# 6Lackiu/EMplanner_Carla

Measured on AMD Instinct MI355X. Metric: planning cycles/sec (DP+QP, 40x9 S-L lattice, 8 obs), higher is better.
Workload: dtype f64

## Files before the change

### emplanner_carla_amd/csrc/emp_dp_kernels.h

```cpp
#pragma once

#include <hip/hip_runtime.h>

#include "emp_core.h"
#include "emp_dp_launch.h"

namespace emp {

__device__ __forceinline__ double jerk_unit_sum(const double* tail, double s0) {
    Quintic u;
    u.a0 = u.a1 = u.a2 = 0.0;
    u.a3 = tail[kSamples + kSampleMoments + 0];
    u.a4 = tail[kSamples + kSampleMoments + 1];
    u.a5 = tail[kSamples + kSampleMoments + 2];
    return jerk_quirk_sum(u, s0, tail[kSamples], tail[kSamples + 1]);
}

__global__ __launch_bounds__(256) void dp_pair_table_kernel(DpDev P, double* __restrict__ tab) {
    const int row = P.row, rr = P.row * P.row;
    for (int p = threadIdx.x; p < rr; p += blockDim.x) {
        const int k = p / row, i = p - k * row;
        const double l_pre = lattice_l(row, k, P.sample_l);
        const double l_cur = lattice_l(row, i, P.sample_l);
        const Quintic q = quintic_shifted(l_pre, 0.0, 0.0, l_cur, P.sample_s);
        double S_l = 0.0, S_dl = 0.0, S_ddl = 0.0;
        for (int n = 0; n < kSamples; ++n) {
            const double t = sample_t(n, P.sample_s);
            const double l = quintic_l(q, t);
            const double dl = quintic_dl(q, t);
            const double ddl = quintic_ddl(q, t);
            tab[n * rr + p] = l;
            S_l = S_l + l * l;
            S_dl = S_dl + dl * dl;
            S_ddl = S_ddl + ddl * ddl;
        }
        const double h = l_cur - l_pre;
        tab[kF_JERK * rr + p] = P.w2 * (h * h);
        tab[kF_BASE * rr + p] = P.w0 * S_dl + P.w1 * S_ddl;
        tab[kF_REF * rr + p] = P.w_ref * S_l;
        tab[kF_LLO * rr + p] = fmin(l_pre, l_cur);
        tab[kF_LHI * rr + p] = fmax(l_pre, l_cur);
    }
    if (threadIdx.x < kSamples) tab[kTableFields * rr + threadIdx.x] = sample_t(threadIdx.x, P.sample_s);
    if (threadIdx.x == 0) {
        sample_moments(P.sample_s, &tab[kTableFields * rr + kSamples], &tab[kTableFields * rr + kSamples + 1]);
        const Quintic u = quintic_shifted(0.0, 0.0, 0.0, 1.0, P.sample_s);
        tab[kTableFields * rr + kSamples + kSampleMoments + 0] = u.a3;
        tab[kTableFields * rr + kSamples + kSampleMoments + 1] = u.a4;
        tab[kTableFields * rr + kSamples + kSampleMoments + 2] = u.a5;
    }
}

#ifndef EMP_SOFT_NEWTON_STEPS
#define EMP_SOFT_NEWTON_STEPS 1
#endif
__device__ __forceinline__ double soft_cost_quotient(double d2) {
    double r = __builtin_amdgcn_rcp(d2);
    r = __builtin_fma(r, __builtin_fma(-d2, r, 1.0), r);
    if (EMP_SOFT_NEWTON_STEPS > 1) r = __builtin_fma(r, __builtin_fma(-d2, r, 1.0), r);
    const double q = kSoftGain * r;
    return __builtin_fma(__builtin_fma(-d2, q, kSoftGain), r, q);
}

#ifndef EMP_SCAN_GROUP
#define EMP_SCAN_GROUP 10
#endif
__device__ __forceinline__ double obstacle_scan_dense(double s0, const double* t_smp, const double* l_n, int stride,
                                                      double os, double ol, double w_coll) {
    double c = 0.0;
    bool alive = true;
#pragma unroll
    for (int g = 0; g < kSamples; g += EMP_SCAN_GROUP) {
        double d2[EMP_SCAN_GROUP];
#pragma unroll
        for (int n = 0; n < EMP_SCAN_GROUP; ++n) {
            const double d_lon = os - (s0 + t_smp[g + n]);
            const double d_lat = ol - l_n[(g + n) * stride];
            d2[n] = d_lon * d_lon + d_lat * d_lat;
        }
#pragma unroll
        for (int n = 0; n < EMP_SCAN_GROUP; ++n) {
            const bool near = alive & (d2[n] < kSafe2);
            const bool hard = near & (d2[n] <= kDanger2);
            if (near & !hard) {
#if EMP_SOFT_NEWTON_STEPS == 1
                asm volatile("");
#endif
                c = c + soft_cost_quotient(d2[n]);
            }
            alive = alive & !hard;
        }
    }
    if (!alive) c = c + w_coll;
    return c;
}

__device__ __forceinline__ bool obstacle_box_in_reach(double os, double ol, double s0, double s9, double l_lo, double l_hi) {
    const double dx = fmax(fmax(s0 - os, os - s9), 0.0);
    const double dy = fmax(fmax(l_lo - ol, ol - l_hi), 0.0);
    return dx * dx + dy * dy < 36.5;
}

template <int ROW = 0, typename MASK = unsigned long long, typename Store>
__device__ __forceinline__ void dp_edge_column(const DpDev& P, int j, int i, double ps, int nob, const double* tab,
                                               const double* t_smp, const double* my_obs_s, const double* my_obs_l,
                                               Store&& store, double* box_dx2 = nullptr) {
    constexpr int kMaskBits = (int)sizeof(MASK) * 8;
    const int row = ROW > 0 ? ROW : P.row, rr = row * row;
    const int nmask = min(nob, kMaskBits);
    const double s0 = ps + (double)j * P.sample_s;
    const double s9 = s0 + t_smp[kSamples - 1];
    const double F = jerk_unit_sum(t_smp, s0);
    MASK near_s = 0;
    for (int m = 0; m < nmask; ++m) {
        const double os = my_obs_s[m];
        if (os > s0 - 6.5 && os < s9 + 6.5) near_s |= (MASK)1 << m;
    }
    if (box_dx2) {
        for (int m = i; m < nmask; m += row) {
            const double os = my_obs_s[m];
            const double dx = fmax(fmax(s0 - os, os - s9), 0.0);
            box_dx2[m] = dx * dx;
        }
        __builtin_amdgcn_wave_barrier();
    }
    for (int k = 0; k < row; ++k) {
        const int p = k * row + i;
        const double smooth = tab[kF_BASE * rr + p] + tab[kF_JERK * rr + p] * F;
        const double l_lo = tab[kF_LLO * rr + p], l_hi = tab[kF_LHI * rr + p];
        double coll = 0.0;
        for (MASK rest = near_s; rest; rest &= rest - 1) {
            const int m = (kMaskBits == 32 ? __ffs((int)rest) : __ffsll((long long)rest)) - 1;
            const double ol = my_obs_l[m];
            if (box_dx2) {
                const double dy = fmax(fmax(l_lo - ol, ol - l_hi), 0.0);
                if (!(box_dx2[m] + dy * dy < 36.5)) continue;
                coll = coll + obstacle_scan_dense(s0, t_smp, &tab[p], rr, my_obs_s[m], ol, P.w_coll);
                continue;
            }
            const double os = my_obs_s[m];
            if (!obstacle_box_in_reach(os, ol, s0, s9, l_lo, l_hi)) continue;
            coll = coll + obstacle_scan_dense(s0, t_smp, &tab[p], rr, os, ol, P.w_coll);
        }
        for (int m = kMaskBits; m < nob; ++m) {
            const double os = my_obs_s[m], ol = my_obs_l[m];
            if (!obstacle_in_reach(os, ol, s0, s9, l_lo, l_hi)) continue;
            coll = coll + obstacle_scan_dense(s0, t_smp, &tab[p], rr, os, ol, P.w_coll);
        }
        store(k, (smooth + coll) + tab[kF_REF * rr + p]);
    }
    if (box_dx2) __builtin_amdgcn_wave_barrier();
}

#ifndef EMP_EDGE_WAVES
#define EMP_EDGE_WAVES 5
#endif
template <bool TILED, int ROW = 0, typename MASK = unsigned long long>
__global__ __launch_bounds__(1024, EMP_EDGE_WAVES) void dp_edge_kernel(DpDev P, const double* __restrict__ pair_tab,
                                                      const double* __restrict__ obs_s,
                                                      const double* __restrict__ obs_l,
                                                      const int* __restrict__ n_obs,
                                                      const double* __restrict__ start,
                                                      double* __restrict__ start_cost,
                                                      double* __restrict__ edge, int cols_per_chunk) {
    extern __shared__ __attribute__((aligned(16))) double lds[];
    __builtin_amdgcn_s_setprio(EMP_PRIO_FRONT);
    const int row = ROW > 0 ? ROW : P.row, rr = row * row;
    double* tab = lds;
    double* t_obs_s = lds + kTableFields * rr;
    double* t_obs_l = t_obs_s + P.S * P.max_obs;
    double* t_smp = t_obs_l + P.S * P.max_obs;
    const int box_w = min(P.max_obs, (int)sizeof(MASK) * 8);
    double* box_all = t_smp + kTableTail;
    const int tile = blockIdx.x;
    const int tid = threadIdx.x;

    for (int x = tid; x < kTableFields * rr; x += blockDim.x) tab[x] = pair_tab[x];
    if (tid < kTableTail) t_smp[tid] = pair_tab[kTableFields * rr + tid];
    for (int x = tid; x < P.S * P.max_obs; x += blockDim.x) {
        const int s = x / P.max_obs, m = x - s * P.max_obs;
        const int b = tile * P.S + s;
        t_obs_s[x] = (b < P.B) ? obs_s[(size_t)b * P.max_obs + m] : 0.0;
        t_obs_l[x] = (b < P.B) ? obs_l[(size_t)b * P.max_obs + m] : 0.0;
    }
    __syncthreads();

    const int lanes_used = P.S * row;

    if (blockIdx.y == 0 && start_cost != nullptr && tid < lanes_used) {
        const int s = tid / row, i = tid - s * row;
        const int b = tile * P.S + s;
        if (b < P.B) {
            const double ps = start[b * 4 + 0], pl = start[b * 4 + 1], pdl = start[b * 4 + 2],
                         pddl = start[b * 4 + 3];
            const Quintic q = quintic_shifted(pl, pdl, pddl, lattice_l(row, i, P.sample_l), P.sample_s);
            start_cost[(size_t)b * row + i] =
                segment_cost(q, ps, P.sample_s, t_obs_s + s * P.max_obs, t_obs_l + s * P.max_obs, min(max(n_obs[b], 0), P.max_obs),
                             P.w_coll, P.w0, P.w1, P.w2, P.w_ref);
        }
    }

    const int j_begin = 1 + blockIdx.y * cols_per_chunk;
    const int j_end = min(P.col, j_begin + cols_per_chunk);
    const int lane = tid & 63;
    const int s = lane / row, i = lane - s * row;
    const int b = tile * P.S + s;
    if (lane >= lanes_used || b >= P.B) return;
    const double ps = start[b * 4 + 0];
    const int nob = min(max(n_obs[b], 0), P.max_obs);
    const double* my_obs_s = t_obs_s + s * P.max_obs;
    const double* my_obs_l = t_obs_l + s * P.max_obs;
    double* my_box = box_all + ((size_t)(tid >> 6) * P.S + s) * box_w;
    for (int j = j_begin + (tid >> 6); j < j_end; j += (int)(blockDim.x >> 6)) {
        dp_edge_column<ROW, MASK>(P, j, i, ps, nob, tab, pair_tab + kTableFields * rr, my_obs_s, my_obs_l, [&](int k, double cost) {
            if (TILED) {
                edge[(((size_t)tile * (P.col - 1) + (j - 1)) * row + k) * 64 + lane] = cost;
            } else {
                edge[(size_t)b * (P.col - 1) * rr + (size_t)(j - 1) * rr + i * row + k] = cost;
            }
        }, my_box);
    }
}

#ifndef EMP_EDGE_RING_BOUNDS
#define EMP_EDGE_RING_BOUNDS __launch_bounds__(1024, EMP_EDGE_WAVES)
#endif
#ifndef EMP_EDGE_NO_SCAN
#define EMP_EDGE_NO_SCAN 0
#endif
constexpr bool kEdgeNoScan = EMP_DEV_HOOKS && EMP_EDGE_NO_SCAN;
template <bool TILED, int ROW = 0, typename MASK = unsigned>
__global__ EMP_EDGE_RING_BOUNDS void dp_edge_ring_kernel(DpDev P, const double* __restrict__ pair_tab,
                                                           const double* __restrict__ obs_s,
                                                           const double* __restrict__ obs_l,
                                                           const int* __restrict__ n_obs,
                                                           const double* __restrict__ start,
                                                           double* __restrict__ start_cost,
                                                           double* __restrict__ edge, int cols_per_chunk,
                                                           unsigned long long* __restrict__ clock_probe = nullptr) {
    extern __shared__ __attribute__((aligned(16))) double lds[];
    __builtin_amdgcn_s_setprio(EMP_PRIO_FRONT);
    const unsigned long long probe_r0 = clock_probe ? wall_clock64() : 0;
    const unsigned long long probe_c0 = clock_probe ? clock64() : 0;
    constexpr int kMaskBits = (int)sizeof(MASK) * 8;
    const int row = ROW > 0 ? ROW : P.row, rr = row * row;
    double* tab = lds;
    double* t_obs_s = lds + kTableFields * rr;
    double* t_obs_l = t_obs_s + P.S * P.max_obs;
    double* t_ps = t_obs_l + P.S * P.max_obs;
    double* box_all = t_ps + ((P.S + 1) & ~1);
    const int waves = (int)(blockDim.x >> 6);
    unsigned char* rings = reinterpret_cast<unsigned char*>(box_all + (size_t)waves * 2 * P.S * P.max_obs);
    const int mask_bytes = edge_ring_mask_bytes(P.max_obs);
    const int cpw = (cols_per_chunk + waves - 1) / waves;
    double* f_all = reinterpret_cast<double*>(rings + (size_t)waves * edge_ring_bytes(P.max_obs));
    const double* t_smp = pair_tab + kTableFields * rr;
    const int tile = blockIdx.x;
    const int tid = threadIdx.x;

    for (int x = tid; x < kTableFields * rr; x += blockDim.x) tab[x] = pair_tab[x];
    for (int x = tid; x < P.S * P.max_obs; x += blockDim.x) {
        const int sc = x / P.max_obs, m = x - sc * P.max_obs;
        const int bb = tile * P.S + sc;
        t_obs_s[x] = (bb < P.B) ? obs_s[(size_t)bb * P.max_obs + m] : 0.0;
        t_obs_l[x] = (bb < P.B) ? obs_l[(size_t)bb * P.max_obs + m] : 0.0;
    }
    if (tid < P.S) t_ps[tid] = (tile * P.S + tid < P.B) ? start[(size_t)(tile * P.S + tid) * 4 + 0] : 0.0;
    __syncthreads();

    const int lanes_used = P.S * row;
    if (blockIdx.y == 0 && start_cost != nullptr && tid < lanes_used) {
        const int sc = tid / row, ii = tid - sc * row;
        const int bb = tile * P.S + sc;
        if (bb < P.B) {
            const double ps0 = start[bb * 4 + 0], pl = start[bb * 4 + 1], pdl = start[bb * 4 + 2], pddl = start[bb * 4 + 3];
            const Quintic q = quintic_shifted(pl, pdl, pddl, lattice_l(row, ii, P.sample_l), P.sample_s);
            start_cost[(size_t)bb * row + ii] =
                segment_cost(q, ps0, P.sample_s, t_obs_s + sc * P.max_obs, t_obs_l + sc * P.max_obs, min(max(n_obs[bb], 0), P.max_obs),
                             P.w_coll, P.w0, P.w1, P.w2, P.w_ref);
        }
    }

    const int j_begin = 1 + blockIdx.y * cols_per_chunk;
    const int j_end = min(P.col, j_begin + cols_per_chunk);
    const int lane = tid & 63;
    const int wave = __builtin_amdgcn_readfirstlane(tid >> 6);
    const int s = lane / row, i = lane - s * row;
    const int b = tile * P.S + s;
    const bool live = (lane < lanes_used) && (b < P.B);
    const int sl = live ? s : 0;
    const double ps = t_ps[sl];
    const int nob = live ? min(min(max(n_obs[b], 0), P.max_obs), kMaskBits) : 0;
    const double* my_obs_s = t_obs_s + sl * P.max_obs;
    const double* my_obs_l = t_obs_l + sl * P.max_obs;
    double* my_band = box_all + ((size_t)wave * P.S + sl) * 2 * P.max_obs;
    unsigned* r_code = reinterpret_cast<unsigned*>(rings + (size_t)wave * edge_ring_bytes(P.max_obs));
    unsigned char* r_mask = reinterpret_cast<unsigned char*>(r_code + 2 * kRingSlots);
    auto put_mask = [&](int slot, MASK v) {
        if (mask_bytes == 1) r_mask[slot] = (unsigned char)v;
        else if (mask_bytes == 2) reinterpret_cast<unsigned short*>(r_mask)[slot] = (unsigned short)v;
        else if (mask_bytes == 4) reinterpret_cast<unsigned*>(r_mask)[slot] = (unsigned)v;
        else reinterpret_cast<unsigned long long*>(r_mask)[slot] = (unsigned long long)v;
    };
    auto get_mask = [&](int slot) -> MASK {
        if (mask_bytes == 1) return (MASK)r_mask[slot];
        if (mask_bytes == 2) return (MASK) reinterpret_cast<const unsigned short*>(r_mask)[slot];
        if (mask_bytes == 4) return (MASK) reinterpret_cast<const unsigned*>(r_mask)[slot];
        return (MASK) reinterpret_cast<const unsigned long long*>(r_mask)[slot];
    };
    double* f_tab = f_all + (size_t)wave * cpw * P.S;
    const float inv_waves = 1.0f / (float)waves;
    int head[2] = {0, 0}, cnt[2] = {0, 0};
    const bool packed = kMaskBits == 32 && mask_bytes <= 2;
    constexpr bool kAhead = TILED && kMaskBits == 32;

    auto store_edge = [&](int j, int k, int owner, double cost) {
        if (TILED) {
            edge[(((size_t)tile * (P.col - 1) + (j - 1)) * row + k) * 64 + owner] = cost;
        } else {
            const int so = owner / row, io = owner - so * row;
            edge[(size_t)(tile * P.S + so) * (P.col - 1) * rr + (size_t)(j - 1) * rr + io * row + k] = cost;
        }
    };
    auto round = [&](int c) {
        const int n = min(cnt[c], 64);
        if (lane < n) {
            const int slot = (head[c] + lane) & (kRingSlots - 1);
            const unsigned code = r_code[c * kRingSlots + slot];
            const int owner = (int)(code & 63u), k = (int)((code >> 12) & 31u), j = (int)(code >> 17);
            const int so = owner / row, io = owner - so * row;
            const int p = k * row + io;
            const double s0 = t_ps[so] + (double)j * P.sample_s;
            const int it = __float2int_rn((float)(j - j_begin - wave) * inv_waves);
            const double smooth = tab[kF_BASE * rr + p] + tab[kF_JERK * rr + p] * f_tab[it * P.S + so];
            const double* o_s = t_obs_s + so * P.max_obs;
            const double* o_l = t_obs_l + so * P.max_obs;
            double coll = 0.0;
            if (kEdgeNoScan) {
            } else if (c == 0) {
                const int m = (int)((code >> 6) & 63u);
                coll = coll + obstacle_scan_dense(s0, t_smp, &tab[p], rr, o_s[m], o_l[m], P.w_coll);
            } else {
                for (MASK rest = get_mask(slot); rest; rest &= rest - 1) {
                    const int m = (kMaskBits == 32 ? __ffs((int)rest) : __ffsll((long long)rest)) - 1;
                    coll = coll + obstacle_scan_dense(s0, t_smp, &tab[p], rr, o_s[m], o_l[m], P.w_coll);
                }
            }
            store_edge(j, k, owner, (smooth + coll) + tab[kF_REF * rr + p]);
        }
        head[c] = (head[c] + n) & (kRingSlots - 1);
        cnt[c] -= n;
        __builtin_amdgcn_wave_barrier();
    };

    for (int j = j_begin + wave; j < j_end; j += waves) {
        const double s0 = ps + (double)j * P.sample_s;
        const double s9 = s0 + t_smp[kSamples - 1];
        MASK near_s = 0, near_w = 0;
        const int my_first_lane = sl * row;
        const unsigned long long row_bits = (1ull << row) - 1;
        for (int m0 = 0; m0 < P.max_obs && m0 < kMaskBits; m0 += row) {
            const int m = m0 + i;
            bool in_reach = false;
            if (live && m < nob) {
                const double os = my_obs_s[m], ol = my_obs_l[m];
                const double dx = fmax(fmax(s0 - os, os - s9), 0.0);
                const double thr = 36.5 - dx * dx;
                const double r = sqrt(fmax(thr, 0.0));
                in_reach = thr > 0.0;
                my_band[2 * m] = in_reach ? ol - r : __builtin_inf();
                my_band[2 * m + 1] = in_reach ? ol + r : -__builtin_inf();
            }
            const unsigned long long votes = __ballot(in_reach);
            const unsigned long long verdicts = (votes >> my_first_lane) & row_bits;
            near_s |= (MASK)((MASK)verdicts << m0);
            unsigned long long any = 0;
            for (int f = 0; f < lanes_used; f += row) any |= votes >> f;
            near_w |= (MASK)((MASK)(any & row_bits) << m0);
        }
        if (!live) near_s = 0;
        __builtin_amdgcn_wave_barrier();
        MASK a_own = 0, b_own = 0;
        {
            const double l_own = tab[kF_LHI * rr + i * row + i];
            for (MASK rest = near_w; rest; rest &= rest - 1) {
                const int m = (kMaskBits == 32 ? __ffs((int)rest) : __ffsll((long long)rest)) - 1;
                const double b_lo = my_band[2 * m], b_hi = my_band[2 * m + 1];
                a_own |= (l_own > b_lo) ? (MASK)1 << m : (MASK)0;
                b_own |= (l_own < b_hi) ? (MASK)1 << m : (MASK)0;
            }
        }
        const double F = jerk_unit_sum(t_smp, s0);
        if (live && i == 0) f_tab[((j - j_begin - wave) / waves) * P.S + s] = F;
        const unsigned x_own = kMaskBits == 32 && packed ? (unsigned)a_own | ((unsigned)b_own << 16) : (unsigned)a_own;
        const unsigned code_j = (unsigned)j << 17;
        unsigned x_k = 0;
        if constexpr (kAhead) x_k = (unsigned)__builtin_amdgcn_ds_bpermute(my_first_lane << 2, (int)x_own);
        for (int k = 0; k < row; ++k) {
            const int p = k * row + i;
            const double t_base = tab[kF_BASE * rr + p], t_jerk = tab[kF_JERK * rr + p], t_ref = tab[kF_REF * rr + p];
            const int src = (my_first_lane + k) << 2;
            if constexpr (!kAhead) x_k = (unsigned)__builtin_amdgcn_ds_bpermute(src, (int)x_own);
            const unsigned u = x_k | x_own;
            if constexpr (kAhead) x_k = (unsigned)__builtin_amdgcn_ds_bpermute((my_first_lane + min(k + 1, row - 1)) << 2, (int)x_own);
            MASK pass;
            if constexpr (kMaskBits == 32) {
                unsigned v = u >> 16;
                if (!packed) v = (unsigned)__builtin_amdgcn_ds_bpermute(src, (int)b_own) | (unsigned)b_own;
                pass = u & v & near_s;
            } else {
                const MASK a_k = ((MASK)(unsigned)__builtin_amdgcn_ds_bpermute(src, (int)(unsigned)(a_own >> 32)) << 32) | u;
                const MASK b_k = ((MASK)(unsigned)__builtin_amdgcn_ds_bpermute(src, (int)(unsigned)(b_own >> 32)) << 32) |
                                 (MASK)(unsigned)__builtin_amdgcn_ds_bpermute(src, (int)(unsigned)b_own);
                pass = (a_k | a_own) & (b_k | b_own) & near_s;
            }
            if (live && pass == 0) store_edge(j, k, lane, ((t_base + t_jerk * F) + 0.0) + t_ref);
            const MASK more = pass & (pass - 1);
            const unsigned long long b_any = __ballot(pass != 0), b2 = __ballot(more != 0), b1 = b_any & ~b2;
            if (b_any) {
                const int before1 = __builtin_amdgcn_mbcnt_hi((unsigned)(b1 >> 32), __builtin_amdgcn_mbcnt_lo((unsigned)b1, 0));
                const int before2 = __builtin_amdgcn_mbcnt_hi((unsigned)(b2 >> 32), __builtin_amdgcn_mbcnt_lo((unsigned)b2, 0));
                const unsigned code_jk = code_j | ((unsigned)k << 12);
                if (pass != 0) {
                    const bool many = more != 0;
                    const int slot = (many ? head[1] + cnt[1] + before2 : head[0] + cnt[0] + before1) & (kRingSlots - 1);
                    const int m1 = (kMaskBits == 32 ? __ffs((int)pass) : __ffsll((long long)pass)) - 1;
                    r_code[slot | (many ? kRingSlots : 0)] = code_jk | ((unsigned)m1 << 6) | (unsigned)lane;
                    if (many) put_mask(slot, pass);
                }
                cnt[0] += __popcll(b1);
                cnt[1] += __popcll(b2);
                __builtin_amdgcn_wave_barrier();
                if (cnt[0] >= 64) round(0);
                if (cnt[1] >= 64) round(1);
            }
        }
        __builtin_amdgcn_wave_barrier();
    }
    while (cnt[0] > 0) round(0);
    while (cnt[1] > 0) round(1);
    if (clock_probe && lane == 0) {
        unsigned long long* o = clock_probe + ((size_t)(blockIdx.y * gridDim.x + blockIdx.x) * waves + wave) * 4;
        o[0] = probe_r0;
        o[1] = wall_clock64();
        o[2] = probe_c0;
        o[3] = clock64();
    }
}

template <int ROW, int PD, int WPB, bool NT = false, bool BT = true>
__global__ __launch_bounds__(64 * WPB) void dp_sweep_kernel(DpDev P, const double* __restrict__ start_cost,
                                                       const double* __restrict__ edge,
                                                       const int* __restrict__ n_obs,
                                                       double* __restrict__ rows_out,
                                                       double* __restrict__ min_cost_out,
                                                       int* __restrict__ status_out,
                                                       unsigned char* __restrict__ pre_out = nullptr,
                                                       int* __restrict__ term_out = nullptr,
                                                       unsigned long long* __restrict__ clock_probe = nullptr) {
    extern __shared__ __attribute__((aligned(16))) unsigned char pre_lds[];
    unsigned long long probe_c0 = 0, probe_r0 = 0;
    if (clock_probe) {
        probe_c0 = clock64();
        probe_r0 = wall_clock64();
    }
    auto probe_end = [&](int tile_, int lane_) {
        if (clock_probe && lane_ == 0) {
            unsigned long long* o = clock_probe + (size_t)tile_ * 4;
            o[0] = probe_c0;
            o[1] = clock64();
            o[2] = probe_r0;
            o[3] = wall_clock64();
        }
    };
    __builtin_amdgcn_s_setprio(EMP_PRIO_SWEEP);
    const int row = ROW > 0 ? ROW : P.row;
    const int wave = threadIdx.x >> 6, lane = threadIdx.x & 63;
    double* cost_lds = reinterpret_cast<double*>(pre_lds);
    const int tile = blockIdx.x * WPB + wave;
    if (tile >= P.tiles) return;
    unsigned char* pre = pre_lds + (size_t)WPB * 64 * sizeof(double) + (size_t)wave * P.col * 64;
    const int s = lane / row, i = lane - s * row;
    const int b = tile * P.S + s;
    const bool live = (lane < P.S * row) && (b < P.B);
    const int base = s * row;
    const bool left = i < (row >> 1);
    const double INF = __builtin_inf();
    const double pen = left ? kLanePenalty : 0.0;

    double cost = INF;
    if (live) {
        cost = start_cost[(size_t)b * row + i];
        if (left) cost = cost + kLanePenalty;
    }
    const double* tile_edge = edge + (size_t)tile * (P.col - 1) * row * 64 + lane;

    double* front = cost_lds + wave * 64;
    auto publish = [&]() {
        front[lane] = cost;
        __builtin_amdgcn_wave_barrier();
    };
    auto relax_one = [&](double e, int k, double& best, int& arg) {
        const double ck = front[base + k];
        double cand = ck + e;
        if (left) cand = cand + kLanePenalty;
        if (cand < best) {
            best = cand;
            arg = k;
        }
    };

    if constexpr (ROW > 0) {
        const int last_col = P.col - 1;
        double ring[PD][ROW];
        auto load_col = [&](double (&dst)[ROW], int jcol) {
            if (last_col < 1) return;
            const int j = min(jcol, last_col);
            const double* src = tile_edge + (size_t)(j - 1) * ROW * 64;
#pragma unroll
            for (int k = 0; k < ROW; ++k) dst[k] = NT ? __builtin_nontemporal_load(&src[k * 64]) : src[k * 64];
        };
        double held[ROW], held_best = INF;
        int held_j = 0;
#pragma unroll
        for (int k = 0; k < ROW; ++k) held[k] = INF;
        auto settle = [&]() {
            int arg = ROW - 1;
#pragma unroll
            for (int k = ROW - 2; k >= 0; --k) arg = (held[k] == held_best) ? k : arg;
            if (held_j > 0) pre[held_j * 64 + lane] = (unsigned char)((held_best < INF) ? arg : 1);
        };
        auto relax_col = [&](const double (&e)[ROW], int j) {
            publish();
            double cand[ROW];
#pragma unroll
            for (int k = 0; k < ROW; ++k) cand[k] = front[base + k];
            settle();
#pragma unroll
            for (int k = 0; k < ROW; ++k) cand[k] = (cand[k] + e[k]) + pen;
            double tree[ROW];
#pragma unroll
            for (int k = 0; k < ROW; ++k) tree[k] = cand[k];
#pragma unroll
            for (int span = 1; span < ROW; span <<= 1) {
#pragma unroll
                for (int k = 0; k + span < ROW; k += 2 * span) tree[k] = __builtin_fmin(tree[k], tree[k + span]);
            }
            cost = __builtin_fmin(tree[0], INF);
#pragma unroll
            for (int k = 0; k < ROW; ++k) held[k] = cand[k];
            held_best = cost;
            held_j = j;
        };
#pragma unroll
        for (int d = 0; d < PD; ++d) load_col(ring[d], 1 + d);
        for (int j0 = 1; j0 < P.col; j0 += PD) {
#pragma unroll
            for (int d = 0; d < PD; ++d) {
                if (j0 + d < P.col) relax_col(ring[d], j0 + d);
                load_col(ring[d], j0 + d + PD);
            }
        }
        settle();
    } else {
        for (int j = 1; j < P.col; ++j) {
            double best = INF;
            int arg = 1;
            publish();
            for (int k = 0; k < row; ++k) relax_one(tile_edge[((size_t)(j - 1) * row + k) * 64], k, best, arg);
            cost = best;
            pre[j * 64 + lane] = (unsigned char)arg;
        }
    }

    double best = INF;
    int arg = 0;
    bool first = true;
    publish();
    for (int k = 0; k < row; ++k) {
        const double ck = front[base + k];
        if (first || ck < best) {
            best = ck;
            arg = k;
            first = false;
        }
    }
    __builtin_amdgcn_wave_barrier();
    if constexpr (!BT) {
        if (live && i == 0) {
            const bool bypass = (n_obs != nullptr) && (n_obs[b] <= 0);
            term_out[b] = arg;
            if (min_cost_out) min_cost_out[b] = bypass ? INF : best;
            status_out[b] = (!bypass && best > P.w_coll) ? 1 : 0;
        }
        const uint4* src = reinterpret_cast<const uint4*>(pre);
        uint4* dst = reinterpret_cast<uint4*>(pre_out + (size_t)tile * P.col * 64);
        for (int w = lane; w < P.col * 4; w += 64) dst[w] = src[w];
        probe_end(tile, lane);
        return;
    }
    if (live && i == 0) {
        const bool bypass = (n_obs != nullptr) && (n_obs[b] <= 0);
        double* out = rows_out + (size_t)b * P.col;
        if (bypass) {
            const double centre = (double)(row + 1) / 2.0 - 1.0;
            for (int j = 0; j < P.col; ++j) out[j] = centre;
            if (min_cost_out) min_cost_out[b] = INF;
            status_out[b] = 0;
        } else {
            int idx = arg;
            out[P.col - 1] = (double)idx;
            for (int j = P.col - 1; j >= 1; --j) {
                idx = pre[j * 64 + base + idx];
                out[j - 1] = (double)idx;
            }
            if (min_cost_out) min_cost_out[b] = best;
            status_out[b] = (best > P.w_coll) ? 1 : 0;
        }
    }
    probe_end(tile, lane);
}


__global__ __launch_bounds__(256) void dp_edge_wide_kernel(DpDev P, const double* __restrict__ pair_tab,
                                                           const double* __restrict__ obs_s, const double* __restrict__ obs_l,
                                                           const int* __restrict__ n_obs, const double* __restrict__ start,
                                                           double* __restrict__ start_cost, double* __restrict__ edge) {
    const int row = P.row;
    const size_t rr = (size_t)P.row * P.row;
    const int b = blockIdx.x, j = 1 + blockIdx.y;
    const int nob = min(max(n_obs[b], 0), P.max_obs);
    const double* my_obs_s = obs_s + (size_t)b * P.max_obs;
    const double* my_obs_l = obs_l + (size_t)b * P.max_obs;
    for (int i = threadIdx.x; i < row; i += blockDim.x) {
        if (blockIdx.y == 0 && start_cost != nullptr) {
            const double ps = start[b * 4 + 0], pl = start[b * 4 + 1], pdl = start[b * 4 + 2], pddl = start[b * 4 + 3];
            const Quintic q = quintic_shifted(pl, pdl, pddl, lattice_l(row, i, P.sample_l), P.sample_s);
            start_cost[(size_t)b * row + i] = segment_cost(q, ps, P.sample_s, my_obs_s, my_obs_l, nob, P.w_coll, P.w0, P.w1, P.w2, P.w_ref);
        }
        if (j >= P.col) continue;
        const double* t_smp = pair_tab + (size_t)kTableFields * rr;
        double* out = edge + (size_t)b * (P.col - 1) * rr + (size_t)(j - 1) * rr + (size_t)i * row;
        dp_edge_column(P, j, i, start[b * 4 + 0], nob, pair_tab, t_smp, my_obs_s, my_obs_l, [&](int k, double cost) { out[k] = cost; });
    }
}

__global__ __launch_bounds__(256) void dp_sweep_wide_kernel(DpDev P, const double* __restrict__ start_cost,
                                                            const double* __restrict__ edge, const int* __restrict__ n_obs,
                                                            unsigned short* __restrict__ pre, double* __restrict__ rows_out,
                                                            double* __restrict__ min_cost_out, int* __restrict__ status_out) {
    extern __shared__ double front_lds[];
    const int row = P.row;
    const size_t rr = (size_t)P.row * P.row;
    const int b = blockIdx.x;
    const double INF = __builtin_inf();
    double* cur = front_lds;
    double* nxt = front_lds + row;
    for (int i = threadIdx.x; i < row; i += blockDim.x) {
        double c = start_cost[(size_t)b * row + i];
        if (i < (row >> 1)) c = c + kLanePenalty;
        cur[i] = c;
    }
    __syncthreads();
    unsigned short* my_pre = pre + (size_t)b * P.col * row;
    for (int j = 1; j < P.col; ++j) {
        const double* ej = edge + (size_t)b * (P.col - 1) * rr + (size_t)(j - 1) * rr;
        for (int i = threadIdx.x; i < row; i += blockDim.x) {
            const bool left = i < (row >> 1);
            double best = INF;
            int arg = 1;
            for (int k = 0; k < row; ++k) {
                double cand = cur[k] + ej[(size_t)i * row + k];
                if (left) cand = cand + kLanePenalty;
                if (cand < best) {
                    best = cand;
                    arg = k;
                }
            }
            nxt[i] = best;
            my_pre[(size_t)j * row + i] = (unsigned short)arg;
        }
        __syncthreads();
        double* t = cur;
        cur = nxt;
        nxt = t;
    }
    if (threadIdx.x == 0) {
        const bool bypass = (n_obs != nullptr) && (n_obs[b] <= 0);
        double* out = rows_out + (size_t)b * P.col;
        if (bypass) {
            const double centre = (double)(row + 1) / 2.0 - 1.0;
            for (int j = 0; j < P.col; ++j) out[j] = centre;
            if (min_cost_out) min_cost_out[b] = INF;
            status_out[b] = 0;
        } else {
            double best = INF;
            int arg = 0;
            bool first = true;
            for (int k = 0; k < row; ++k) {
                const double ck = cur[k];
                if (first || ck < best) {
                    best = ck;
                    arg = k;
                    first = false;
                }
            }
            int idx = arg;
            out[P.col - 1] = (double)idx;
            for (int j = P.col - 1; j >= 1; --j) {
                idx = my_pre[(size_t)j * row + idx];
                out[j - 1] = (double)idx;
            }
            if (min_cost_out) min_cost_out[b] = best;
            status_out[b] = (best > P.w_coll) ? 1 : 0;
        }
    }
}


template <int ROW>
__global__ __launch_bounds__(256, 4) void dp_fused_kernel(DpDev P, const double* __restrict__ pair_tab,
                                                          const double* __restrict__ obs_s,
                                                          const double* __restrict__ obs_l,
                                                          const int* __restrict__ n_obs,
                                                          const double* __restrict__ start,
                                                          double* __restrict__ rows_out,
                                                          double* __restrict__ min_cost_out,
                                                          int* __restrict__ status_out, int nc) {
    extern __shared__ __attribute__((aligned(16))) double lds[];
    const int row = ROW > 0 ? ROW : P.row, rr = row * row;
    const FusedLds L = fused_lds(row, P.col, P.S, P.max_obs, nc);
    unsigned char* base_b = reinterpret_cast<unsigned char*>(lds);
    double* tab = lds;
    double* t_smp = reinterpret_cast<double*>(base_b + L.off_smp);
    double* t_obs_s = reinterpret_cast<double*>(base_b + L.off_obs_s);
    double* t_obs_l = reinterpret_cast<double*>(base_b + L.off_obs_l);
    double* buf = reinterpret_cast<double*>(base_b + L.off_buf);
    double* front = reinterpret_cast<double*>(base_b + L.off_front);
    unsigned char* pre = base_b + L.off_pre;
    int* ctr = reinterpret_cast<int*>(base_b + L.off_ctr);
    const int tile = blockIdx.x, tid = threadIdx.x, lane = tid & 63;
    const int wave = __builtin_amdgcn_readfirstlane(tid >> 6);

    for (int x = tid; x < kTableFields * rr; x += blockDim.x) tab[x] = pair_tab[x];
    if (tid < kTableTail) t_smp[tid] = pair_tab[kTableFields * rr + tid];
    for (int x = tid; x < P.S * P.max_obs; x += blockDim.x) {
        const int sc = x / P.max_obs, m = x - sc * P.max_obs;
        const int bb = tile * P.S + sc;
        t_obs_s[x] = (bb < P.B) ? obs_s[(size_t)bb * P.max_obs + m] : 0.0;
        t_obs_l[x] = (bb < P.B) ? obs_l[(size_t)bb * P.max_obs + m] : 0.0;
    }
    if (tid < 2) ctr[tid] = 0;
    __syncthreads();

    const int s = lane / row, i = lane - s * row;
    const int b = tile * P.S + s;
    const bool live = (lane < P.S * row) && (b < P.B);
    const int sl = live ? s : 0;
    const double ps = live ? start[b * 4 + 0] : 0.0;
    const int nob = live ? min(max(n_obs[b], 0), P.max_obs) : 0;
    const double* my_obs_s = t_obs_s + sl * P.max_obs;
    const double* my_obs_l = t_obs_l + sl * P.max_obs;
    const int base = s * row;
    const bool left = i < (row >> 1);
    const double INF = __builtin_inf();
    const double pen = left ? kLanePenalty : 0.0;

    double cost = INF;
    constexpr int HR = ROW > 0 ? ROW : 1;
    double held[HR], held_best = INF;
    int held_j = 0;
#pragma unroll
    for (int k = 0; k < HR; ++k) held[k] = INF;
    auto publish = [&]() {
        front[lane] = cost;
        __builtin_amdgcn_wave_barrier();
    };
    auto settle = [&]() {
        if constexpr (ROW > 0) {
            int arg = ROW - 1;
#pragma unroll
            for (int k = ROW - 2; k >= 0; --k) arg = (held[k] == held_best) ? k : arg;
            if (held_j > 0) pre[held_j * 64 + lane] = (unsigned char)((held_best < INF) ? arg : 1);
        }
    };
    auto relax_col = [&](const double* e , int j) {
        if constexpr (ROW > 0) {
            publish();
            double cand[ROW];
#pragma unroll
            for (int k = 0; k < ROW; ++k) cand[k] = front[base + k];
            settle();
#pragma unroll
            for (int k = 0; k < ROW; ++k) cand[k] = (cand[k] + e[k * 64]) + pen;
            double tree[ROW];
#pragma unroll
            for (int k = 0; k < ROW; ++k) tree[k] = cand[k];
#pragma unroll
            for (int span = 1; span < ROW; span <<= 1) {
#pragma unroll
                for (int k = 0; k + span < ROW; k += 2 * span) tree[k] = __builtin_fmin(tree[k], tree[k + span]);
            }
            cost = __builtin_fmin(tree[0], INF);
#pragma unroll
            for (int k = 0; k < ROW; ++k) held[k] = cand[k];
            held_best = cost;
            held_j = j;
        } else {
            double best = INF;
            int arg = 1;
            publish();
            for (int k = 0; k < row; ++k) {
                double cand = front[base + k] + e[k * 64];
                if (left) cand = cand + kLanePenalty;
                if (cand < best) {
                    best = cand;
                    arg = k;
                }
            }
            cost = best;
            pre[j * 64 + lane] = (unsigned char)arg;
        }
    };

    if (wave == 0 && live) {
        const Quintic q = quintic_shifted(start[b * 4 + 1], start[b * 4 + 2], start[b * 4 + 3], lattice_l(row, i, P.sample_l),
                                          P.sample_s);
        cost = segment_cost(q, ps, P.sample_s, my_obs_s, my_obs_l, nob, P.w_coll, P.w0, P.w1, P.w2, P.w_ref);
        if (left) cost = cost + kLanePenalty;
    }

    const int ncol = P.col - 1;
    const int nchunks = (ncol + nc - 1) / nc;
    for (int c = 0; c < nchunks; ++c) {
        const int par = c & 1;
        const int j0 = 1 + c * nc;
        const int cols = min(nc, P.col - j0);
        double* cbuf = buf + (size_t)par * nc * row * 64;
        if (tid == 0) ctr[par ^ 1] = 0;
        for (;;) {
            int jj = 0;
            if (lane == 0) jj = atomicAdd(&ctr[par], 1);
            jj = __builtin_amdgcn_readfirstlane(jj);
            if (jj >= cols) break;
            double* dst = cbuf + (size_t)jj * row * 64 + lane;
            if (live) dp_edge_column(P, j0 + jj, i, ps, nob, tab, t_smp, my_obs_s, my_obs_l, [&](int k, double v) { dst[k * 64] = v; });
        }
        __syncthreads();
        if (wave == 0)
            for (int jj = 0; jj < cols; ++jj) relax_col(cbuf + (size_t)jj * row * 64 + lane, j0 + jj);
    }
    if (wave != 0) return;
    settle();

    double best = INF;
    int arg = 0;
    bool first = true;
    publish();
    for (int k = 0; k < row; ++k) {
        const double ck = front[base + k];
        if (first || ck < best) {
            best = ck;
            arg = k;
            first = false;
        }
    }
    __builtin_amdgcn_wave_barrier();
    if (live && i == 0) {
        const bool bypass = n_obs[b] <= 0;
        double* out = rows_out + (size_t)b * P.col;
        if (bypass) {
            const double centre = (double)(row + 1) / 2.0 - 1.0;
            for (int j = 0; j < P.col; ++j) out[j] = centre;
            if (min_cost_out) min_cost_out[b] = INF;
            status_out[b] = 0;
        } else {
            int idx = arg;
            out[P.col - 1] = (double)idx;
            for (int j = P.col - 1; j >= 1; --j) {
                idx = pre[j * 64 + base + idx];
                out[j - 1] = (double)idx;
            }
            if (min_cost_out) min_cost_out[b] = best;
            status_out[b] = (best > P.w_coll) ? 1 : 0;
        }
    }
}

__global__ __launch_bounds__(64) void dp_enrich_wave_kernel(DpDev P, const double* __restrict__ rows,
                                                           const double* __restrict__ start, int max_pts,
                                                           double* __restrict__ path_s, double* __restrict__ path_l,
                                                           int* __restrict__ path_len, int* __restrict__ status,
                                                           int or_status, const unsigned char* __restrict__ pre = nullptr,
                                                           const int* __restrict__ term = nullptr,
                                                           const int* __restrict__ n_obs = nullptr,
                                                           double* __restrict__ rows_out = nullptr) {
    extern __shared__ __attribute__((aligned(16))) double enrich_lds[];
    const int b = blockIdx.x, lane = threadIdx.x & 63;
    const double ps = start[b * 4 + 0];
    double* os = path_s + (size_t)b * max_pts;
    double* ol = path_l + (size_t)b * max_pts;
    double* lrows = enrich_lds;
    const double* my_rows = lrows;
    if (pre == nullptr) {
        for (int j = lane; j < P.col; j += 64) lrows[j] = rows[(size_t)b * P.col + j];
        __syncthreads();
    } else {
        unsigned char* bt = reinterpret_cast<unsigned char*>(lrows + P.col);
        const int tile = b / P.S, base = (b - tile * P.S) * P.row;
        const unsigned char* tp = pre + (size_t)tile * P.col * 64 + base;
        for (int j = 1 + lane; j < P.col; j += 64)
            for (int r = 0; r < P.row; ++r) bt[j * P.row + r] = tp[j * 64 + r];
        __syncthreads();
        if (lane == 0) {
            if (n_obs != nullptr && n_obs[b] <= 0) {
                const double centre = (double)(P.row + 1) / 2.0 - 1.0;
                for (int j = 0; j < P.col; ++j) lrows[j] = centre;
            } else {
                int idx = term[b];
                lrows[P.col - 1] = (double)idx;
                for (int j = P.col - 1; j >= 1; --j) {
                    idx = bt[j * P.row + idx];
                    lrows[j - 1] = (double)idx;
                }
            }
        }
        __syncthreads();
        for (int j = lane; j < P.col; j += 64) rows_out[(size_t)b * P.col + j] = lrows[j];
    }
    int n_before = 0;
    bool trunc = false;
    double last_s = ps, last_l = start[b * 4 + 1];
    for (int c0 = 0; c0 < P.col; c0 += 64) {
        const int c = c0 + lane;
        const bool in = c < P.col;
        const int cc = in ? c : P.col - 1;
        const double s0 = (cc == 0) ? ps : ps + (double)cc * P.sample_s;
        const double end_s = ps + (double)(cc + 1) * P.sample_s;
        const double l0 = (cc == 0) ? start[b * 4 + 1] : lattice_l_f(P.row, my_rows[cc - 1], P.sample_l);
        const double dl0 = (cc == 0) ? start[b * 4 + 2] : 0.0, ddl0 = (cc == 0) ? start[b * 4 + 3] : 0.0;
        const double end_l = lattice_l_f(P.row, my_rows[cc], P.sample_l);
        const double span = end_s - s0;
        const int cnt = in ? arange_count(span, P.res) : 0;
        int incl = cnt;
#pragma unroll
        for (int d = 1; d < 64; d <<= 1) {
            const int v = __shfl_up(incl, d, 64);
            if (lane >= d) incl += v;
        }
        const int off = n_before + incl - cnt;
        const Quintic q = quintic_shifted(l0, dl0, ddl0, end_l, span);
        for (int k = 0; k < cnt; ++k) {
            const double t = (double)k * P.res;
            const int n = off + k;
            if (n < max_pts) {
                os[n] = s0 + t;
                ol[n] = quintic_l(q, t);
            } else {
                trunc = true;
            }
        }
        n_before += __shfl(incl, 63, 64);
        const int owner = min(P.col - 1 - c0, 63);
        last_s = __shfl(end_s, owner, 64);
        last_l = __shfl(end_l, owner, 64);
    }
    int n = n_before;
    if (n < max_pts) {
        if (lane == 0) {
            os[n] = last_s;
            ol[n] = last_l;
        }
        ++n;
    } else {
        trunc = true;
    }
    n = min(n, max_pts);
    for (int k = n + lane; k < max_pts; k += 64) {
        os[k] = 0.0;
        ol[k] = 0.0;
    }
    const bool any_trunc = __any(trunc);
    if (lane == 0) {
        path_len[b] = n;
        if (or_status) {
            if (any_trunc) status[b] |= 32;
        } else {
            status[b] = any_trunc ? 32 : 0;
        }
    }
}

__global__ void enrich_nodes_kernel(int B, int max_nodes, double res, const double* __restrict__ node_s,
                                    const double* __restrict__ node_l, const int* __restrict__ n_nodes,
                                    const double* __restrict__ start, int max_pts, double* __restrict__ path_s,
                                    double* __restrict__ path_l, int* __restrict__ path_len, int* __restrict__ status) {
    const int b = blockIdx.x * blockDim.x + threadIdx.x;
    if (b >= B) return;
    double s0 = start[b * 4 + 0], l0 = start[b * 4 + 1], dl0 = start[b * 4 + 2], ddl0 = start[b * 4 + 3];
    double* os = path_s + (size_t)b * max_pts;
    double* ol = path_l + (size_t)b * max_pts;
    int n = 0;
    bool trunc = false;
    double end_s = s0, end_l = l0;
    const int cols = min(max(n_nodes[b], 0), max_nodes);
    for (int c = 0; c < cols; ++c) {
        end_s = node_s[(size_t)b * max_nodes + c];
        end_l = node_l[(size_t)b * max_nodes + c];
        const double span = end_s - s0;
        const int cnt = arange_count(span, res);
        const Quintic q = quintic_shifted(l0, dl0, ddl0, end_l, span);
        for (int k = 0; k < cnt; ++k) {
            const double t = (double)k * res;
            if (n < max_pts) {
                os[n] = s0 + t;
                ol[n] = quintic_l(q, t);
                ++n;
            } else {
                trunc = true;
            }
        }
        s0 = end_s;
        l0 = end_l;
        dl0 = 0.0;
        ddl0 = 0.0;
    }
    if (cols > 0) {
        if (n < max_pts) {
            os[n] = end_s;
            ol[n] = end_l;
            ++n;
        } else {
            trunc = true;
        }
    }
    path_len[b] = n;
    status[b] = trunc ? 32 : 0;
}

}
```

Baseline: 18.66 million.

## Precompute source-point obstacle hits to skip dense collision scans for certain edges

Adds a per-lane mask of obstacles that sit within the danger radius of an edge's first sample point. Such obstacles are known hits, so their cost is added as a constant weight without running the dense sample scan. Edges whose only candidates are known hits are stored directly, and single-scan edges carry hit flags in the ring code so the flush adds the weights before and after the scan in order. It also forces the jerk tail coefficients into scalar registers. The price is an extra ballot per obstacle chunk, an extra permute when the hit mask does not fit in the packed word, more branching, and a dependence on the first-sample hit exactly matching what the scan would give.

Result: faster. 19.27 million, median of 6 (+3.3%).

```diff
diff --git a/emplanner_carla_amd/csrc/emp_dp_kernels.h b/emplanner_carla_amd/csrc/emp_dp_kernels.h
--- a/emplanner_carla_amd/csrc/emp_dp_kernels.h
+++ b/emplanner_carla_amd/csrc/emp_dp_kernels.h
@@ -313,6 +313,10 @@
     int head[2] = {0, 0}, cnt[2] = {0, 0};
     const bool packed = kMaskBits == 32 && mask_bytes <= 2;
     constexpr bool kAhead = TILED && kMaskBits == 32;
+    constexpr bool kSrcHit = kAhead && ROW > 0;
+    const bool hit_in_word = packed && mask_bytes == 1, hit_word = packed && mask_bytes == 2;
+    const double w_hit_v = 0.0 + P.w_coll;
+    const double w_hit = __hiloint2double(__builtin_amdgcn_readfirstlane(__double2hiint(w_hit_v)), __builtin_amdgcn_readfirstlane(__double2loint(w_hit_v)));
 
     auto store_edge = [&](int j, int k, int owner, double cost) {
         if (TILED) {
@@ -338,8 +342,12 @@
             double coll = 0.0;
             if (kEdgeNoScan) {
             } else if (c == 0) {
-                const int m = (int)((code >> 6) & 63u);
+                const unsigned mf = (code >> 6) & 63u;
+                const bool flags = kSrcHit && packed;
+                const int m = (int)(flags ? mf & 15u : mf);
+                if (flags && (mf & 16u)) coll = coll + w_hit;
                 coll = coll + obstacle_scan_dense(s0, t_smp, &tab[p], rr, o_s[m], o_l[m], P.w_coll);
+                if (flags && (mf & 32u)) coll = coll + w_hit;
             } else {
                 for (MASK rest = get_mask(slot); rest; rest &= rest - 1) {
                     const int m = (kMaskBits == 32 ? __ffs((int)rest) : __ffsll((long long)rest)) - 1;
@@ -357,17 +365,22 @@
         const double s0 = ps + (double)j * P.sample_s;
         const double s9 = s0 + t_smp[kSamples - 1];
         MASK near_s = 0, near_w = 0;
+        MASK hit_w = 0;
         const int my_first_lane = sl * row;
         const unsigned long long row_bits = (1ull << row) - 1;
         for (int m0 = 0; m0 < P.max_obs && m0 < kMaskBits; m0 += row) {
             const int m = m0 + i;
-            bool in_reach = false;
+            bool in_reach = false, cand = false;
             if (live && m < nob) {
                 const double os = my_obs_s[m], ol = my_obs_l[m];
                 const double dx = fmax(fmax(s0 - os, os - s9), 0.0);
                 const double thr = 36.5 - dx * dx;
                 const double r = sqrt(fmax(thr, 0.0));
                 in_reach = thr > 0.0;
+                if constexpr (kSrcHit) if (packed) {
+                    const double d_lon = os - (s0 + t_smp[0]);
+                    cand = in_reach && d_lon * d_lon <= kDanger2;
+                }
                 my_band[2 * m] = in_reach ? ol - r : __builtin_inf();
                 my_band[2 * m + 1] = in_reach ? ol + r : -__builtin_inf();
             }
@@ -377,32 +390,62 @@
             unsigned long long any = 0;
             for (int f = 0; f < lanes_used; f += row) any |= votes >> f;
             near_w |= (MASK)((MASK)(any & row_bits) << m0);
+            if constexpr (kSrcHit) if (packed) {
+                const unsigned long long hv = __ballot(cand);
+                unsigned long long hany = 0;
+                if (hv) for (int f = 0; f < lanes_used; f += row) hany |= hv >> f;
+                hit_w |= (MASK)((MASK)(hany & row_bits) << m0);
+            }
         }
         if (!live) near_s = 0;
         __builtin_amdgcn_wave_barrier();
-        MASK a_own = 0, b_own = 0;
+        MASK a_own = 0, b_own = 0, h_own = 0;
         {
             const double l_own = tab[kF_LHI * rr + i * row + i];
+            const double l_src = tab[i * row + i];
+            const double s_src = s0 + t_smp[0];
             for (MASK rest = near_w; rest; rest &= rest - 1) {
                 const int m = (kMaskBits == 32 ? __ffs((int)rest) : __ffsll((long long)rest)) - 1;
                 const double b_lo = my_band[2 * m], b_hi = my_band[2 * m + 1];
                 a_own |= (l_own > b_lo) ? (MASK)1 << m : (MASK)0;
                 b_own |= (l_own < b_hi) ? (MASK)1 << m : (MASK)0;
             }
-        }
-        const double F = jerk_unit_sum(t_smp, s0);
+            if constexpr (kSrcHit) {
+                for (MASK rest = hit_w; rest; rest &= rest - 1) {
+                    const int m = (kMaskBits == 32 ? __ffs((int)rest) : __ffsll((long long)rest)) - 1;
+                    const double d_lon = my_obs_s[m] - s_src, d_lat = my_obs_l[m] - l_src;
+                    h_own |= (d_lon * d_lon + d_lat * d_lat <= kDanger2) ? (MASK)1 << m : (MASK)0;
+                }
+                h_own &= near_s;
+            }
+        }
+        double F;
+        if constexpr (kSrcHit) {
+            double tail[kTableTail];
+#pragma unroll
+            for (int n = 0; n < kTableTail; ++n) tail[n] = t_smp[n];
+            asm volatile("" : "+s"(tail[kSamples + kSampleMoments + 0]), "+s"(tail[kSamples + kSampleMoments + 1]),
+                              "+s"(tail[kSamples + kSampleMoments + 2]));
+            F = jerk_unit_sum(tail, s0);
+        } else {
+            F = jerk_unit_sum(t_smp, s0);
+        }
         if (live && i == 0) f_tab[((j - j_begin - wave) / waves) * P.S + s] = F;
-        const unsigned x_own = kMaskBits == 32 && packed ? (unsigned)a_own | ((unsigned)b_own << 16) : (unsigned)a_own;
+        const unsigned x_own = kMaskBits == 32 && packed ? (unsigned)a_own | ((unsigned)b_own << 16) | (hit_in_word ? (unsigned)h_own << 8 : 0u)
+                                                         : (unsigned)a_own;
         const unsigned code_j = (unsigned)j << 17;
-        unsigned x_k = 0;
+        unsigned x_k = 0, hx_k = 0;
         if constexpr (kAhead) x_k = (unsigned)__builtin_amdgcn_ds_bpermute(my_first_lane << 2, (int)x_own);
+        if constexpr (kSrcHit) if (hit_word) hx_k = (unsigned)__builtin_amdgcn_ds_bpermute(my_first_lane << 2, (int)(unsigned)h_own);
         for (int k = 0; k < row; ++k) {
             const int p = k * row + i;
             const double t_base = tab[kF_BASE * rr + p], t_jerk = tab[kF_JERK * rr + p], t_ref = tab[kF_REF * rr + p];
             const int src = (my_first_lane + k) << 2;
             if constexpr (!kAhead) x_k = (unsigned)__builtin_amdgcn_ds_bpermute(src, (int)x_own);
             const unsigned u = x_k | x_own;
+            const unsigned h_k = hit_in_word ? (x_k >> 8) & 0xffu : hx_k;
             if constexpr (kAhead) x_k = (unsigned)__builtin_amdgcn_ds_bpermute((my_first_lane + min(k + 1, row - 1)) << 2, (int)x_own);
+            if constexpr (kSrcHit) if (hit_word) hx_k = (unsigned)__builtin_amdgcn_ds_bpermute((my_first_lane + min(k + 1, row - 1)) << 2, (int)(unsigned)h_own);
             MASK pass;
             if constexpr (kMaskBits == 32) {
                 unsigned v = u >> 16;
@@ -414,17 +457,34 @@
                                  (MASK)(unsigned)__builtin_amdgcn_ds_bpermute(src, (int)(unsigned)b_own);
                 pass = (a_k | a_own) & (b_k | b_own) & near_s;
             }
-            if (live && pass == 0) store_edge(j, k, lane, ((t_base + t_jerk * F) + 0.0) + t_ref);
-            const MASK more = pass & (pass - 1);
-            const unsigned long long b_any = __ballot(pass != 0), b2 = __ballot(more != 0), b1 = b_any & ~b2;
+            MASK scan = pass;
+            if constexpr (kSrcHit) {
+                scan = pass & ~(MASK)h_k;
+                if (live && scan == 0) {
+                    double coll = 0.0;
+                    for (int n = __popc((unsigned)pass); n > 0; --n) coll = coll + w_hit;
+                    store_edge(j, k, lane, ((t_base + t_jerk * F) + coll) + t_ref);
+                }
+            } else {
+                if (live && pass == 0) store_edge(j, k, lane, ((t_base + t_jerk * F) + 0.0) + t_ref);
+            }
+            MASK more = scan != 0 ? pass & (pass - 1) : (MASK)0;
+            unsigned m_flags = 0;
+            if constexpr (kSrcHit) {
+                const unsigned hb = pass & ~scan, below = hb & (scan - 1), above = hb ^ below;
+                const bool one = ((scan & (scan - 1)) | (below & (below - 1)) | (above & (above - 1))) == 0;
+                more = (scan != 0 && !one) ? 1u : 0u;
+                m_flags = (below ? 16u : 0u) | (above ? 32u : 0u);
+            }
+            const unsigned long long b_any = __ballot(scan != 0), b2 = __ballot(more != 0), b1 = b_any & ~b2;
             if (b_any) {
                 const int before1 = __builtin_amdgcn_mbcnt_hi((unsigned)(b1 >> 32), __builtin_amdgcn_mbcnt_lo((unsigned)b1, 0));
                 const int before2 = __builtin_amdgcn_mbcnt_hi((unsigned)(b2 >> 32), __builtin_amdgcn_mbcnt_lo((unsigned)b2, 0));
                 const unsigned code_jk = code_j | ((unsigned)k << 12);
-                if (pass != 0) {
+                if (scan != 0) {
                     const bool many = more != 0;
                     const int slot = (many ? head[1] + cnt[1] + before2 : head[0] + cnt[0] + before1) & (kRingSlots - 1);
-                    const int m1 = (kMaskBits == 32 ? __ffs((int)pass) : __ffsll((long long)pass)) - 1;
+                    const int m1 = (int)m_flags | ((kMaskBits == 32 ? __ffs((int)scan) : __ffsll((long long)scan)) - 1);
                     r_code[slot | (many ? kRingSlots : 0)] = code_jk | ((unsigned)m1 << 6) | (unsigned)lane;
                     if (many) put_mask(slot, pass);
                 }
```
